# wischmcj/pyQSM

Measured on AMD Instinct MI355X. Metric: Mpoints/s DBSCAN (1M-pt synthetic forest, eps=0.1, min_neighbors=10), higher is better.
Workload: dtype f64; 1 GPU; 1000000-point synthetic tree cloud (configs[1]), DBSCAN eps=0.1 min_neighbors=10, 20 clusters; replicas at N>1; points_per_gpu=1000000, parallelism=replicas x1

## Files before the change

pyqsm_amd/csrc/grid.hip:

```cpp
#include "grid.hpp"

#include <atomic>
#include <cmath>
#include <type_traits>

namespace pyqsm {

__device__ __forceinline__ unsigned long long ord_key(double x) {
  unsigned long long b = static_cast<unsigned long long>(__double_as_longlong(x));
  return (b >> 63) ? ~b : (b | 0x8000000000000000ull);
}
static double ord_val(unsigned long long k) {
  unsigned long long b = (k >> 63) ? (k & 0x7FFFFFFFFFFFFFFFull) : ~k;
  double d;
  memcpy(&d, &b, 8);
  return d;
}

static constexpr int kBoxVals = 7;
__global__ __launch_bounds__(256) void k_bbox(const double* __restrict__ xyz, int64_t n,
                                              unsigned long long* __restrict__ part ,
    unsigned long long* __restrict__ st ) {
  __shared__ unsigned long long red[4][6];
  __shared__ int red_f32[4];
// ... 717 lines not shown
struct BkRec;
template <>
struct BkRec<true> {
  using type = float4;
};
template <>
struct BkRec<false> {
  using type = PointRec;
};

template <int MODE>
__global__ __launch_bounds__(256) void k_bk_hist(const double* __restrict__ xyz, int64_t n, GridParams g,
                                                 int rx, int ry, int rz, AxisMap am, int nbk, int bits,
                                                 int32_t* __restrict__ key_tmp,
                                                 int32_t* __restrict__ tot, const GridPlan* __restrict__ plan) {
  extern __shared__ __attribute__((aligned(16))) int32_t h[];
  if (plan) {
    if (!plan->ok) return;
    g = GridParams{plan->mn[0], plan->mn[1], plan->mn[2], plan->inv_cell, plan->nx, plan->ny, plan->nz};
    rx = plan->rx;
    ry = plan->ry;
    rz = plan->rz;
    nbk = plan->nbk;
    bits = plan->bits;
  }
  for (int b = threadIdx.x; b < nbk; b += 256) h[b] = 0;
  __syncthreads();
  const int64_t base = int64_t(blockIdx.x) * kBkPts;
#pragma unroll
  for (int k = 0; k < kBkPts / 256; ++k) {
    const int64_t i = base + k * 256 + threadIdx.x;
    if (i < n) {
      int c, oct = 0;
      if (MODE == 2) {
        c = cell_index(g, xyz[3 * i], xyz[3 * i + 1], xyz[3 * i + 2]);
      } else {
        const RawCell r = raw_cell(g, rx, ry, rz, xyz[3 * i], xyz[3 * i + 1], xyz[3 * i + 2]);
        const int cx = MODE == 1 ? am.x[r.cx] : r.cx + 1, cy = MODE == 1 ? am.y[r.cy] : r.cy + 1,
                  cz = MODE == 1 ? am.z[r.cz] : r.cz + 1;
        c = (cz * g.ny + cy) * g.nx + cx;
        oct = r.oct;
      }
      key_tmp[i] = (c << 3) | oct;
      atomicAdd(&h[c >> bits], 1);
    }
  }
  __syncthreads();
  for (int b = threadIdx.x; b < nbk; b += 256) {
    const int v = h[b];
    if (v) atomicAdd(&tot[b], v);
  }
}

static constexpr int kBkFusedScan = 4096;
__global__ __launch_bounds__(1024) void k_bk_scan(int nbk, const int32_t* __restrict__ tot,
                                                  int32_t* __restrict__ bstart, const GridPlan* __restrict__ plan) {
  __shared__ int32_t wsum[16];
  if (plan) {
    if (!plan->ok) return;
    nbk = plan->nbk;
  }
  const int per = (nbk + 1023) / 1024;
  const int b0 = threadIdx.x * per;
  int32_t v[16], s = 0;
  for (int k = 0; k < per; ++k) {
    v[k] = b0 + k < nbk ? tot[b0 + k] : 0;
    s += v[k];
  }
  const int lane = threadIdx.x & 63, w = threadIdx.x >> 6;
  int32_t incl = s;
#pragma unroll
  for (int off = 1; off < 64; off <<= 1) {
    const int32_t t = __shfl_up(incl, off, 64);
    if (lane >= off) incl += t;
  }
  if (lane == 63) wsum[w] = incl;
  __syncthreads();
  int32_t run = incl - s;
  for (int q = 0; q < w; ++q) run += wsum[q];
  for (int k = 0; k < per; ++k) {
    if (b0 + k < nbk) bstart[b0 + k] = run;
    run += v[k];
  }
  if (threadIdx.x == 1023) bstart[nbk] = run;
}

template <bool F32>
__global__ __launch_bounds__(256) void k_bk_scatter(const double* __restrict__ xyz, int64_t n, int nbk,
                                                    int bits, const int32_t* __restrict__ key_tmp,
                                                    const int32_t* __restrict__ tot,
                                                    int32_t* __restrict__ cursor ,
                                                    int32_t* __restrict__ bstart ,
                                                    int fused,
                                                    typename BkRec<F32>::type* __restrict__ bucketed,
                                                    int32_t* __restrict__ keyb ,
                                                    const GridPlan* __restrict__ plan) {
  extern __shared__ __attribute__((aligned(16))) int32_t h[];
  const int64_t base = int64_t(blockIdx.x) * kBkPts;
  using Coord = typename std::conditional<F32, float, double>::type;
  int key[kBkPts / 256], lr[kBkPts / 256];
  Coord px[kBkPts / 256], py[kBkPts / 256], pz[kBkPts / 256];
#pragma unroll
  for (int k = 0; k < kBkPts / 256; ++k) {
    const int64_t i = base + k * 256 + threadIdx.x;
    key[k] = -1;
    px[k] = py[k] = pz[k] = Coord(0);
    if (i < n) {
      key[k] = key_tmp[i];
      px[k] = Coord(xyz[3 * i]);
      py[k] = Coord(xyz[3 * i + 1]);
      pz[k] = Coord(xyz[3 * i + 2]);
    }
  }
  if (plan) {
    if (!plan->ok) return;
    nbk = plan->nbk;
    bits = plan->bits;
  }
  int32_t* pre = h + nbk;
  __shared__ int32_t wsum[4];
  for (int b = threadIdx.x; b < nbk; b += 256) h[b] = 0;
  if (fused) {
    constexpr int kPer = kBkFusedScan / 256;
    const int b0 = threadIdx.x * kPer;
    int32_t v[kPer], s = 0;
#pragma unroll
    for (int k = 0; k < kPer; ++k) {
      v[k] = b0 + k < nbk ? tot[b0 + k] : 0;
      s += v[k];
    }
    const int lane = threadIdx.x & 63, w = threadIdx.x >> 6;
    int32_t incl = s;
#pragma unroll
    for (int off = 1; off < 64; off <<= 1) {
      const int32_t t = __shfl_up(incl, off, 64);
      if (lane >= off) incl += t;
    }
    if (lane == 63) wsum[w] = incl;
    __syncthreads();
    int32_t run = incl - s;
    for (int q = 0; q < w; ++q) run += wsum[q];
#pragma unroll
    for (int k = 0; k < kPer; ++k) {
      if (b0 + k < nbk) {
        pre[b0 + k] = run;
        if (blockIdx.x == 0) bstart[b0 + k] = run;
      }
      run += v[k];
    }
    if (blockIdx.x == 0 && threadIdx.x == 255) bstart[nbk] = run;
  }
  __syncthreads();
#pragma unroll
  for (int k = 0; k < kBkPts / 256; ++k) {
    lr[k] = key[k] >= 0 ? atomicAdd(&h[key[k] >> (3 + bits)], 1) : 0;
  }
  __syncthreads();
  for (int bb = 0; bb < nbk; bb += 16 * 256) {
    int32_t v[16], a[16];
#pragma unroll
    for (int k = 0; k < 16; ++k) {
      const int b = bb + k * 256 + threadIdx.x;
      v[k] = b < nbk ? h[b] : 0;
    }
#pragma unroll
    for (int k = 0; k < 16; ++k) {
      a[k] = 0;
      if (v[k]) a[k] = atomicAdd(&cursor[bb + k * 256 + threadIdx.x], v[k]);
    }
#pragma unroll
    for (int k = 0; k < 16; ++k) {
      const int b = bb + k * 256 + threadIdx.x;
      if (v[k]) h[b] = (fused ? pre[b] : bstart[b]) + a[k];
    }
  }
  __syncthreads();
#pragma unroll
  for (int k = 0; k < kBkPts / 256; ++k) {
    if (key[k] < 0) continue;
    const int64_t i = base + k * 256 + threadIdx.x;
    const int pos = h[key[k] >> (3 + bits)] + lr[k];
    keyb[pos] = key[k];
    if constexpr (F32) {
      bucketed[pos] = make_float4(px[k], py[k], pz[k], __int_as_float(int(i)));
    } else {
      PointRec r;
      r.x = px[k];
      r.y = py[k];
      r.z = pz[k];
      r.idx = int(i);
      r.key = key[k];
      bucketed[pos] = r;
    }
  }
}

__device__ __forceinline__ int bytes_below(unsigned long long x, int o) {
  x &= (1ull << (8 * o)) - 1ull;
  x = (x & 0x00FF00FF00FF00FFull) + ((x >> 8) & 0x00FF00FF00FF00FFull);
  x = (x & 0x0000FFFF0000FFFFull) + ((x >> 16) & 0x0000FFFF0000FFFFull);
  return int((x + (x >> 32)) & 0xFFFFull);
}

template <int BITS>
struct BkLds {
  unsigned long long oct[1 << BITS];
  int32_t cnt[1 << BITS];
  uint32_t big[(1 << BITS) / 32];
  int32_t wsum[16];
  int32_t osum[16];
  int32_t any_big;
  int32_t btot[8], bbase[8];
  int32_t bw[(1 << BITS) / 512][8];
};

__device__ __forceinline__ uint32_t bk_word(int lk, int rr, int r8) {
  return (uint32_t(lk) << 16) | (uint32_t(rr < 255 ? rr : 255) << 8) | uint32_t(r8);
}

template <bool F32>
static constexpr int kBkGrp = F32 ? 2 : 1;

template <int BITS, bool F32>
__global__ __launch_bounds__((1 << BITS) / 8, BITS == 12 ? 6 : 4) void k_bk_sort(
    const int32_t* __restrict__ bstart,
    const typename BkRec<F32>::type* __restrict__ bucketed, const int32_t* __restrict__ keyb,
    uint32_t* __restrict__ word_tmp, int32_t* __restrict__ rank_tmp,
    DirWord* __restrict__ words , int32_t* __restrict__ slots ,
    int32_t* __restrict__ order, int32_t* __restrict__ cell_of, int32_t* __restrict__ sub_of,
    double* __restrict__ sx, double* __restrict__ sy, double* __restrict__ sz,
    float4* __restrict__ p4 , int4* __restrict__ rec,
    PointRec* __restrict__ keyed ,
    const GridPlan* __restrict__ plan ,
    unsigned long long* __restrict__ st ) {
  constexpr int CELLS = 1 << BITS, T = CELLS / 8, CAP = T * kBkPer, G = kBkGrp<F32>;
  using Rec = typename BkRec<F32>::type;
  static_assert(kBkPer % G == 0, "whole groups");
  __shared__ BkLds<BITS> L;
  stamped(st, [&] {
  const int bk = blockIdx.x, t = threadIdx.x;
  if (!plan->ok || bk >= plan->nbk) return;
  const int s = bstart[bk], e = bstart[bk + 1];
  const int64_t c0 = int64_t(bk) << BITS;
  constexpr int WORDS = CELLS / 32;
  DirWord* const wds = words + size_t(bk) * WORDS;
  const uint32_t sb = uint32_t(s) + uint32_t(bk);
  if (s == e) {
    if (t < WORDS) wds[t] = DirWord{0u, sb};
    if (t == 0) slots[sb] = s;
    return;
  }
  if (e - s <= 64) {
    int32_t* const cells = L.cnt;
    int32_t* const dcell = L.cnt + 64;
    const int m = e - s;
    if (t < 64) {
      const bool live = t < m;
      const int lk = live ? keyb[s + t] & (8 * CELLS - 1) : 0;
      Rec p = {};
      if (live) p = bucketed[s + t];
      int below_key = 0, below_cell = 0;
      unsigned long long oc = 0ull;
      for (int q = 0; q < m; ++q) {
        const int kq = __builtin_amdgcn_readlane(lk, q);
        below_key += (kq < lk || (kq == lk && q < t)) ? 1 : 0;
        below_cell += (kq >> 3) < (lk >> 3) ? 1 : 0;
        if ((kq >> 3) == (lk >> 3)) oc += 1ull << (8 * (kq & 7));
      }
      if (live) {
        const int cl = lk >> 3, o = lk & 7, b = s + below_cell, f = s + below_key;
        cells[below_key] = cl;
        cell_of[f] = int(c0) + cl;
        sub_of[f] = b * 8 + o;
        if constexpr (F32) {
          order[f] = __float_as_int(p.w);
          p4[f] = make_float4(p.x, p.y, p.z, 0.f);
        } else {
          order[f] = p.idx;
          sx[f] = p.x;
          sy[f] = p.y;
          sz[f] = p.z;
        }
        if (below_key == below_cell) {
          int r2 = b;
#pragma unroll
          for (int o2 = 0; o2 < 8; ++o2) {
            const int cnt = int((oc >> (8 * o2)) & 255ull);
            rec[size_t(b) * 8 + o2] = make_int4(r2, cnt, -1, 0);
            r2 += cnt;
          }
        }
      }
    }
    __syncthreads();
    if (t < 64) {
      const bool live = t < m;
      const int ci = live ? cells[t] : -1;
      const bool head = live && (t == 0 || cells[t - 1] != ci);
      const unsigned long long hm = __ballot(head);
      const int rk = __popcll(hm & ((1ull << t) - 1ull));
      if (head) {
        slots[sb + rk] = s + t;
        dcell[rk] = ci;
      }
      if (t == 0) {
        slots[sb + __popcll(hm)] = e;
        L.wsum[0] = __popcll(hm);
      }
    }
    __syncthreads();
    if (t < WORDS) {
      const int nd = L.wsum[0];
      uint32_t bits = 0u, before = 0u;
      for (int q = 0; q < nd; ++q) {
        const int c = dcell[q];
        before += c < 32 * t ? 1u : 0u;
        bits |= (c >> 5) == t ? 1u << (c & 31) : 0u;
      }
      wds[t] = DirWord{bits, sb + before};
    }
    return;
  }
  uint32_t wd[kBkPer];
#pragma unroll
  for (int k = 0; k < kBkPer; ++k) {
    const int j = s + k * T + t;
    wd[k] = j < e ? uint32_t(keyb[j]) : 0u;
  }
  Rec cur[G] = {};
#pragma unroll
  for (int k = 0; k < G; ++k) {
    const int j = s + k * T + t;
    if (j < e) cur[k] = bucketed[j];
  }
#pragma unroll
  for (int k = 0; k < 8; ++k) {
    L.oct[k * T + t] = 0ull;
    L.cnt[k * T + t] = 0;
  }
  if (t < CELLS / 32) L.big[t] = 0u;
  if (t == 0) L.any_big = 0;
  __syncthreads();
  auto rank_of = [&](uint32_t ky, int j) {
    const int lk = int(ky) & (8 * CELLS - 1), cl = lk >> 3, o = lk & 7;
    const int rr = atomicAdd(&L.cnt[cl], 1);
    const int r8 = int((atomicAdd(&L.oct[cl], 1ull << (8 * o)) >> (8 * o)) & 255ull);
    if (rr >= 255) rank_tmp[j] = rr;
    return bk_word(lk, rr, r8);
  };
#pragma unroll
  for (int k = 0; k < kBkPer; ++k) {
    const int j = s + k * T + t;
    if (j < e) wd[k] = rank_of(wd[k], j);
  }
  for (int base = s + CAP; base < e; base += CAP) {
    uint32_t kk[kBkPer];
#pragma unroll
    for (int k = 0; k < kBkPer; ++k) {
      const int j = base + k * T + t;
      kk[k] = j < e ? uint32_t(keyb[j]) : 0u;
    }
#pragma unroll
    for (int k = 0; k < kBkPer; ++k) {
      const int j = base + k * T + t;
      if (j < e) word_tmp[j] = rank_of(kk[k], j);
    }
  }
  __syncthreads();
  int32_t v[8], tot = 0;
  {
    const int4 a = *reinterpret_cast<const int4*>(&L.cnt[8 * t]);
    const int4 b = *reinterpret_cast<const int4*>(&L.cnt[8 * t + 4]);
    v[0] = a.x; v[1] = a.y; v[2] = a.z; v[3] = a.w;
    v[4] = b.x; v[5] = b.y; v[6] = b.z; v[7] = b.w;
#pragma unroll
    for (int k = 0; k < 8; ++k) tot += v[k];
  }
  uint32_t occ8 = 0u;
#pragma unroll
  for (int k = 0; k < 8; ++k) occ8 |= v[k] ? 1u << k : 0u;
  const int nocc = __popc(occ8);
  const int lane = t & 63, w = t >> 6;
  int32_t incl = tot, oincl = nocc;
#pragma unroll
  for (int off = 1; off < 64; off <<= 1) {
    const int32_t u = __shfl_up(incl, off, 64), uo = __shfl_up(oincl, off, 64);
    if (lane >= off) {
      incl += u;
      oincl += uo;
    }
  }
  if (lane == 63) {
    L.wsum[w] = incl;
    L.osum[w] = oincl;
  }
  __syncthreads();
  int32_t run = incl - tot, orun = oincl - nocc;
  for (int q = 0; q < w; ++q) {
    run += L.wsum[q];
    orun += L.osum[q];
  }
  int32_t pre[8];
#pragma unroll
  for (int k = 0; k < 8; ++k) {
    pre[k] = run;
    run += v[k];
  }
  {
    const uint32_t b1 = __shfl_down(occ8, 1, 64), b2 = __shfl_down(occ8, 2, 64), b3 = __shfl_down(occ8, 3, 64);
    if ((t & 3) == 0) wds[t >> 2] = DirWord{occ8 | (b1 << 8) | (b2 << 16) | (b3 << 24), sb + uint32_t(orun)};
    if (t == T - 1) slots[sb + uint32_t(orun + nocc)] = e;
  }
#pragma unroll
  for (int k = 0; k < 8; ++k) {
    const int cl = 8 * t + k;
    L.cnt[cl] = pre[k];
    if (v[k] == 0) continue;
    const int b = s + pre[k];
    slots[sb + uint32_t(orun) + __popc(occ8 & ((1u << k) - 1u))] = b;
    if (v[k] > kBkBig) {
      atomicOr(&L.big[cl >> 5], 1u << (cl & 31));
      L.any_big = 1;
      continue;
    }
    const unsigned long long c64 = L.oct[cl];
    int r2 = b;
#pragma unroll
    for (int o = 0; o < 8; ++o) {
      const int cnt = int((c64 >> (8 * o)) & 255ull);
      rec[size_t(b) * 8 + o] = make_int4(r2, cnt, -1, 0);
      r2 += cnt;
    }
  }
  __syncthreads();
  auto place = [&](const Rec& p, uint32_t w, int j) {
    const int lk = int(w >> 16), cl = lk >> 3, o = lk & 7, arr = int((w >> 8) & 255u);
    const int b = s + L.cnt[cl];
    if ((L.big[cl >> 5] >> (cl & 31)) & 1u) {
      PointRec q;
      q.x = p.x;
      q.y = p.y;
      q.z = p.z;
      q.key = int(c0 << 3) + lk;
      if constexpr (F32)
        q.idx = __float_as_int(p.w);
      else
        q.idx = p.idx;
      keyed[b + (arr < 255 ? arr : rank_tmp[j])] = q;
      return;
    }
    const int f = b + bytes_below(L.oct[cl], o) + int(w & 255u);
    cell_of[f] = int(c0) + cl;
    sub_of[f] = b * 8 + o;
    if constexpr (F32) {
      order[f] = __float_as_int(p.w);
      p4[f] = make_float4(p.x, p.y, p.z, 0.f);
    } else {
      order[f] = p.idx;
      sx[f] = p.x;
      sy[f] = p.y;
      sz[f] = p.z;
    }
  };
#pragma unroll
  for (int g = 0; g < kBkPer / G; ++g) {
    if (s + g * G * T >= e) break;
    Rec nxt[G] = {};
    if (g + 1 < kBkPer / G) {
#pragma unroll
      for (int k = 0; k < G; ++k) {
        const int j = s + ((g + 1) * G + k) * T + t;
        if (j < e) nxt[k] = bucketed[j];
      }
    }
#pragma unroll
    for (int k = 0; k < G; ++k) {
      const int j = s + (g * G + k) * T + t;
      if (j < e) place(cur[k], wd[g * G + k], j);
    }
#pragma unroll
    for (int k = 0; k < G; ++k) cur[k] = nxt[k];
  }
  for (int base = s + CAP; base < e; base += CAP) {
#pragma unroll
    for (int g = 0; g < kBkPer / G; ++g) {
      if (base + g * G * T >= e) break;
      Rec r[G] = {};
      uint32_t w[G];
#pragma unroll
      for (int k = 0; k < G; ++k) {
        const int j = base + (g * G + k) * T + t;
        w[k] = 0u;
        if (j < e) {
          r[k] = bucketed[j];
          w[k] = word_tmp[j];
        }
      }
#pragma unroll
      for (int k = 0; k < G; ++k) {
        const int j = base + (g * G + k) * T + t;
        if (j < e) place(r[k], w[k], j);
      }
    }
  }
  __syncthreads();
  if (!L.any_big) return;
  for (int wd = 0; wd < CELLS / 32; ++wd) {
    for (uint32_t bm = L.big[wd]; bm; bm &= bm - 1u) {
      const int cl = wd * 32 + __ffs(bm) - 1;
      const int b = s + L.cnt[cl], e2 = s + (cl + 1 < CELLS ? L.cnt[cl + 1] : e - s);
      int loc[8] = {0, 0, 0, 0, 0, 0, 0, 0};
      for (int q = b + t; q < e2; q += T) {
        const int oq = keyed[q].key & 7;
#pragma unroll
        for (int k = 0; k < 8; ++k) loc[k] += oq == k;
      }
      if (t < 8) L.btot[t] = 0;
      __syncthreads();
#pragma unroll
      for (int k = 0; k < 8; ++k) {
        int cnt = loc[k];
        for (int off = 32; off > 0; off >>= 1) cnt += __shfl_down(cnt, off, 64);
        if (lane == 0 && cnt) atomicAdd(&L.btot[k], cnt);
      }
      __syncthreads();
      if (t == 0) {
        int r2 = b;
        for (int k = 0; k < 8; ++k) {
          L.bbase[k] = r2;
          rec[size_t(b) * 8 + k] = make_int4(r2, L.btot[k], -1, 0);
          r2 += L.btot[k];
        }
      }
      __syncthreads();
      for (int q0 = b; q0 < e2; q0 += T) {
        const int q = q0 + t;
        const bool live = q < e2;
        PointRec pr;
        pr.key = 0;
        if (live) pr = keyed[q];
        const int o = pr.key & 7;
        int before = 0;
#pragma unroll
        for (int k = 0; k < 8; ++k) {
          const unsigned long long m = __ballot(live && o == k);
          if (lane == 0) L.bw[w][k] = __popcll(m);
          if (o == k) before = __popcll(m & ((1ull << lane) - 1ull));
        }
        __syncthreads();
        if (live) {
          int f = L.bbase[o] + before;
          for (int ww = 0; ww < w; ++ww) f += L.bw[ww][o];
          order[f] = pr.idx;
          cell_of[f] = pr.key >> 3;
          sub_of[f] = b * 8 + o;
          if (p4) {
            p4[f] = make_float4(float(pr.x), float(pr.y), float(pr.z), 0.f);
          } else {
            sx[f] = pr.x;
            sy[f] = pr.y;
            sz[f] = pr.z;
          }
        }
        __syncthreads();
        if (t < 8) {
          int add = 0;
          for (int ww = 0; ww < T / 64; ++ww) add += L.bw[ww][t];
          L.bbase[t] += add;
        }
        __syncthreads();
      }
    }
  }
  });
}

template <int BITS, bool F32>
__global__ __launch_bounds__((1 << BITS) / 8, BITS == 12 ? 6 : 4) void k_bk_sort_plain(
    int64_t ncell1, const int32_t* __restrict__ bstart, const typename BkRec<F32>::type* __restrict__ bucketed,
    const int32_t* __restrict__ keyb, uint32_t* __restrict__ word_tmp, int32_t* __restrict__ rank_tmp,
    int32_t* __restrict__ start, int32_t* __restrict__ order,
    int32_t* __restrict__ cell_of, double* __restrict__ sx, double* __restrict__ sy, double* __restrict__ sz,
    float4* __restrict__ p4 , int32_t* __restrict__ occ) {
  constexpr int CELLS = 1 << BITS, T = CELLS / 8, CAP = T * kBkPer, G = kBkGrp<F32>;
  using Rec = typename BkRec<F32>::type;
  __shared__ int32_t cnt[CELLS];
  __shared__ int32_t wsum[16], wocc[16];
  const int bk = blockIdx.x, t = threadIdx.x;
  const int s = bstart[bk], e = bstart[bk + 1];
  const int64_t c0 = int64_t(bk) << BITS;
  if (s == e) {
#pragma unroll
    for (int k = 0; k < 2; ++k) {
      const int64_t cidx = c0 + int64_t(k * T + t) * 4;
      if (cidx + 3 < ncell1) {
        *reinterpret_cast<int4*>(start + cidx) = make_int4(s, s, s, s);
      } else {
        for (int u = 0; u < 4; ++u)
          if (cidx + u < ncell1) start[cidx + u] = s;
      }
    }
    if (t == 0) occ[bk] = 0;
    return;
  }
  constexpr int RB = 32 - BITS;
  constexpr int RMAX = (1 << RB) - 1;
  uint32_t wd[kBkPer];
#pragma unroll
  for (int k = 0; k < kBkPer; ++k) {
    const int j = s + k * T + t;
    wd[k] = j < e ? uint32_t(keyb[j]) : 0u;
  }
  Rec cur[G] = {};
#pragma unroll
  for (int k = 0; k < G; ++k) {
    const int j = s + k * T + t;
    if (j < e) cur[k] = bucketed[j];
  }
#pragma unroll
  for (int k = 0; k < 8; ++k) cnt[k * T + t] = 0;
  __syncthreads();
  auto rank_of = [&](uint32_t ky, int j) {
    const int cl = int(ky >> 3) & (CELLS - 1);
    const int rr = atomicAdd(&cnt[cl], 1);
    if (rr >= RMAX) rank_tmp[j] = rr;
    return (uint32_t(cl) << RB) | uint32_t(rr < RMAX ? rr : RMAX);
// ... 84 lines not shown
  };
#pragma unroll
  for (int g = 0; g < kBkPer / G; ++g) {
    if (s + g * G * T >= e) break;
    Rec nxt[G] = {};
    if (g + 1 < kBkPer / G) {
#pragma unroll
      for (int k = 0; k < G; ++k) {
        const int j = s + ((g + 1) * G + k) * T + t;
        if (j < e) nxt[k] = bucketed[j];
      }
    }
#pragma unroll
    for (int k = 0; k < G; ++k) {
      const int j = s + (g * G + k) * T + t;
      if (j < e) place(cur[k], wd[g * G + k], j);
    }
#pragma unroll
    for (int k = 0; k < G; ++k) cur[k] = nxt[k];
  }
  for (int base = s + CAP; base < e; base += CAP) {
#pragma unroll
    for (int g = 0; g < kBkPer / G; ++g) {
      if (base + g * G * T >= e) break;
      Rec r[G] = {};
      uint32_t w[G];
#pragma unroll
      for (int k = 0; k < G; ++k) {
        const int j = base + (g * G + k) * T + t;
        w[k] = 0u;
        if (j < e) {
          r[k] = bucketed[j];
          w[k] = word_tmp[j];
        }
      }
#pragma unroll
      for (int k = 0; k < G; ++k) {
        const int j = base + (g * G + k) * T + t;
        if (j < e) place(r[k], w[k], j);
      }
    }
  }
}

static bool bucketed_fits(const DevGrid& g) {
  const int bits = g.ncell + 1 <= (int64_t(kBkMax) << 12) ? 12 : 13;
  const int64_t nbk = (g.ncell + (int64_t(1) << bits)) >> bits;
  const char* env = getenv("PYQSM_GRID_BIN");
  return nbk <= kBkMax && !(env && !strcmp(env, "atomic"));
}

static void enqueue_bk_a(Ctx* c, int mode, bool f32, const double* xyz, int64_t n, const GridParams& gp,
                         const int raw[3], AxisMap am, int64_t nbk, int bits, int32_t* key_tmp, int32_t* tot,
                         int32_t* cursor, int32_t* bstart, void* bucketed, int32_t* keyb, const GridPlan* d_plan) {
  const dim3 ga(ceil_div(n, kBkPts)), blk(256);
  const size_t lds = size_t(nbk) * 4;
  const int fused = nbk <= kBkFusedScan;
#define PQ_BK_HIST(MODE)                                                                                         \
  hipLaunchKernelGGL(k_bk_hist<MODE>, ga, blk, lds, c->stream, xyz, n, gp, raw[0], raw[1], raw[2], am, int(nbk), \
                     bits, key_tmp, tot, d_plan)
  if (mode == 0)
    PQ_BK_HIST(0);
  else if (mode == 1)
    PQ_BK_HIST(1);
  else
    PQ_BK_HIST(2);
#undef PQ_BK_HIST
  if (!fused) hipLaunchKernelGGL(k_bk_scan, dim3(1), dim3(1024), 0, c->stream, int(nbk), tot, bstart, d_plan);
  if (f32)
    hipLaunchKernelGGL(k_bk_scatter<true>, ga, blk, fused ? 2 * lds : lds, c->stream, xyz, n, int(nbk), bits,
                       key_tmp, tot, cursor, bstart, fused, static_cast<float4*>(bucketed), keyb, d_plan);
  else
    hipLaunchKernelGGL(k_bk_scatter<false>, ga, blk, fused ? 2 * lds : lds, c->stream, xyz, n, int(nbk), bits,
                       key_tmp, tot, cursor, bstart, fused, static_cast<PointRec*>(bucketed), keyb, d_plan);
}

template <int BITS, bool F32>
static void launch_bk_sort_plain(Ctx* c, int64_t nbk, const int32_t* bstart, const void* bucketed, const int32_t* keyb,
                                 uint32_t* word_tmp, int32_t* rank_tmp, DevGrid* g) {
  hipLaunchKernelGGL((k_bk_sort_plain<BITS, F32>), dim3(unsigned(nbk)), dim3((1 << BITS) / 8), 0, c->stream,
                     g->ncell + 1, bstart, static_cast<const typename BkRec<F32>::type*>(bucketed), keyb, word_tmp,
                     rank_tmp, g->start, g->order, g->cell_of, g->sx, g->sy, g->sz, g->p4, g->occ_part);
}

static int build_grid_bucketed(Ctx* c, const double* xyz, int64_t n, DevGrid* g) {
  const int bits = g->ncell + 1 <= (int64_t(kBkMax) << 12) ? 12 : 13;
  const int64_t nbk = (g->ncell + (int64_t(1) << bits)) >> bits;
  const bool f32 = g->p4 != nullptr;
  int32_t *tot, *bstart, *cursor, *key_tmp, *keyb, *rank_tmp;
  uint32_t* word_tmp;
  void* bucketed;
  PQ_TRY(c->arena.get(size_t(nbk) * 2, &tot));
  cursor = tot + nbk;
  PQ_TRY(c->arena.get(size_t(nbk) + 1, &bstart));
  PQ_TRY(c->arena.get(size_t(n), &key_tmp));
  PQ_TRY(c->arena.get(size_t(n), &keyb));
  PQ_TRY(c->arena.get(size_t(n), &word_tmp));
  PQ_TRY(c->arena.get(size_t(n), &rank_tmp));
  if (f32) {
    float4* b4;
    PQ_TRY(c->arena.get(size_t(n), &b4));
    bucketed = b4;
  } else {
    PointRec* b8;
    PQ_TRY(c->arena.get(size_t(n), &b8));
    bucketed = b8;
  }
  g->occ_blocks = int(nbk);
  PQ_TRY(c->arena.get(size_t(nbk), &g->occ_part));
  PQ_HIP(hipMemsetAsync(tot, 0, size_t(nbk) * 8, c->stream));
  const int raw[3] = {0, 0, 0};
  enqueue_bk_a(c, 2, f32, xyz, n, grid_params(*g), raw, AxisMap{nullptr, nullptr, nullptr}, nbk, bits, key_tmp, tot,
               cursor, bstart, bucketed, keyb, nullptr);
  if (bits == 12) {
    if (f32)
      launch_bk_sort_plain<12, true>(c, nbk, bstart, bucketed, keyb, word_tmp, rank_tmp, g);
    else
      launch_bk_sort_plain<12, false>(c, nbk, bstart, bucketed, keyb, word_tmp, rank_tmp, g);
  } else {
    if (f32)
      launch_bk_sort_plain<13, true>(c, nbk, bstart, bucketed, keyb, word_tmp, rank_tmp, g);
    else
      launch_bk_sort_plain<13, false>(c, nbk, bstart, bucketed, keyb, word_tmp, rank_tmp, g);
  }
  PQ_HIP(hipGetLastError());
  return 0;
}


__device__ __forceinline__ double ord_val_dev(unsigned long long k) {
  const unsigned long long b = (k >> 63) ? (k & 0x7FFFFFFFFFFFFFFFull) : ~k;
  return __longlong_as_double(static_cast<long long>(b));
}

__device__ void write_plan(const unsigned long long* box, const PlanIn& in, GridPlan* __restrict__ plan) {
  GridPlan p;
  bool ok = in.hint.valid != 0;
  for (int a = 0; a < 3; ++a) {
    p.mn[a] = ord_val_dev(box[a]);
    p.mx[a] = ord_val_dev(box[3 + a]);
    ok = ok && isfinite(p.mn[a]) && isfinite(p.mx[a]);
  }
  p.all_f32 = box[6] != 0 ? 1 : 0;
  ok = ok && p.all_f32;
  double tot = 1.0;
  int raw[3];
  for (int a = 0; a < 3; ++a) {
    const double d = floor((p.mx[a] - p.mn[a]) / in.cell) + 1.0;
    if (!(d < 2.0e9)) ok = false;
    raw[a] = ok ? int(d) : 0;
    tot *= d + 2.0;
  }
  ok = ok && tot <= double(in.max_cells);
  p.inv_cell = 1.0 / in.cell;
  p.rx = raw[0];
  p.ry = raw[1];
  p.rz = raw[2];
  p.nx = raw[0] + 2;
  p.ny = raw[1] + 2;
  p.nz = raw[2] + 2;
  const int64_t ncell = ok ? int64_t(p.nx) * p.ny * p.nz : 0;
  const int64_t nbk = (ncell + 4096) >> 12;
  ok = ok && ncell + 1 <= (int64_t(kBkMax) << 12) && ncell <= in.hint.ncell && nbk <= in.hint.nbk &&
       (nbk <= kBkFusedScan) == (in.hint.fused != 0);
  p.ncell = ok ? int(ncell) : 0;
  p.nbk = ok ? int(nbk) : 0;
  p.bits = 12;
  p.ok = ok ? 1 : 0;
  p.seq = in.seq;
  *plan = p;
  if (in.host) {
    p.seq = 0;
    *in.host = p;
    __threadfence_system();
    *reinterpret_cast<volatile unsigned*>(&in.host->seq) = in.seq;
  }
}

int plan_grid_device(Ctx* c, const double* xyz, int64_t n, double cell, int64_t max_cells, const PlanHint& hint,
                     GridPlan* d_plan, GridPlan* h_plan, unsigned seq, int32_t* zero_buf, int zero_n) {
  if (n <= 0) return fail(PYQSM_EINVAL, "bounding box of an empty cloud");
  const int blocks = int(std::min<int64_t>(ceil_div(n, 256), int64_t(c->cu_count) * 4));
  unsigned long long *d_box = nullptr, *d_part = nullptr;
  PQ_TRY(c->arena.get(kBoxVals, &d_box));
  PQ_TRY(c->arena.get(size_t(blocks) * kBoxVals, &d_part));
  hipLaunchKernelGGL(k_bbox, dim3(blocks), dim3(256), 0, c->stream, xyz, n, d_part, stamp_slots(c, blocks));
  hipLaunchKernelGGL(k_bbox_fold, dim3(1), dim3(256), 0, c->stream, d_part, blocks, d_box, zero_buf, zero_n,
                     PlanIn{cell, max_cells, hint, h_plan, seq}, d_plan);
  PQ_HIP(hipGetLastError());
  return 0;
}

int octant_zeroed_ints() { return 2 * kBkMax + 5 + kZeroedExtra; }

template <int BITS, bool F32>
static void launch_bk_sort(Ctx* c, int64_t nbk, const int32_t* bstart, const void* bucketed,
                           const int32_t* keyb, uint32_t* word_tmp, int32_t* rank_tmp, PointRec* keyed,
                           const GridPlan* d_plan, DevGrid* g, SubCells* sub) {
  unsigned long long* const st_sort = stamp_slots(c, nbk);
  hipLaunchKernelGGL((k_bk_sort<BITS, F32>), dim3(unsigned(nbk)), dim3((1 << BITS) / 8), 0, c->stream, bstart,
                     static_cast<const typename BkRec<F32>::type*>(bucketed), keyb, word_tmp, rank_tmp, g->dir_words,
                     g->dir_slots, g->order,
                     g->cell_of, sub->sub_of, g->sx, g->sy, g->sz, g->p4, sub->rec, keyed, d_plan, st_sort);
}

static int enqueue_bucketed(Ctx* c, const double* xyz, int64_t n, const GridParams& gp, const int raw[3],
                            AxisMap am, bool mapped, int64_t nbk, int bits, bool f32,
                            int32_t* zeroed, const GridPlan* d_plan, DevGrid* g, SubCells* sub) {
  int32_t *cell_tmp, *keyb, *rank_tmp, *bstart;
  uint32_t* word_tmp;
  int32_t *tot = zeroed, *cursor = zeroed + kBkMax;
  PointRec* keyed;
  void* bucketed;
  g->p4 = nullptr;
  g->sx = g->sy = g->sz = nullptr;
  sub->sub_cnt = sub->sub_beg = nullptr;
  g->start = nullptr;
  PQ_TRY(c->arena.get(size_t(nbk) << (bits - 5), &g->dir_words));
  PQ_TRY(c->arena.get(size_t(n) + size_t(nbk) + 1, &g->dir_slots));
  PQ_TRY(c->arena.get(size_t(n), &g->order));
  PQ_TRY(c->arena.get(size_t(n), &g->cell_of));
  if (f32) {
    float4* b4;
    PQ_TRY(c->arena.get(size_t(n), &g->p4));
    PQ_TRY(c->arena.get(size_t(n), &b4));
    bucketed = b4;
  } else {
    PointRec* b8;
    PQ_TRY(c->arena.get(size_t(n), &g->sx));
    PQ_TRY(c->arena.get(size_t(n), &g->sy));
    PQ_TRY(c->arena.get(size_t(n), &g->sz));
    PQ_TRY(c->arena.get(size_t(n), &b8));
    bucketed = b8;
  }
  PQ_TRY(c->arena.get(size_t(n), &cell_tmp));
  PQ_TRY(c->arena.get(size_t(n), &keyb));
  PQ_TRY(c->arena.get(size_t(n), &word_tmp));
  PQ_TRY(c->arena.get(size_t(n), &rank_tmp));
  PQ_TRY(c->arena.get(size_t(n), &keyed));
  PQ_TRY(c->arena.get(size_t(n), &sub->sub_of));
  PQ_TRY(c->arena.get(size_t(n) * 8, &sub->rec));
  PQ_TRY(c->arena.get(size_t(nbk) + 1, &bstart));
  enqueue_bk_a(c, mapped ? 1 : 0, f32, xyz, n, gp, raw, am, nbk, bits, cell_tmp, tot, cursor, bstart, bucketed, keyb,
               d_plan);
  if (bits == 12) {
    if (f32)
      launch_bk_sort<12, true>(c, nbk, bstart, bucketed, keyb, word_tmp, rank_tmp, keyed, d_plan, g, sub);
    else
      launch_bk_sort<12, false>(c, nbk, bstart, bucketed, keyb, word_tmp, rank_tmp, keyed, d_plan, g, sub);
  } else {
    if (f32)
      launch_bk_sort<13, true>(c, nbk, bstart, bucketed, keyb, word_tmp, rank_tmp, keyed, d_plan, g, sub);
    else
      launch_bk_sort<13, false>(c, nbk, bstart, bucketed, keyb, word_tmp, rank_tmp, keyed, d_plan, g, sub);
  }
  PQ_HIP(hipGetLastError());
  return 0;
}

__global__ __launch_bounds__(256) void k_dir_from_dense(int64_t ncell, const int32_t* __restrict__ start,
                                                        DirWord* __restrict__ words, int32_t* __restrict__ slots) {
  const int64_t c = int64_t(blockIdx.x) * 256 + threadIdx.x;
  const int lane = threadIdx.x & 63, half = lane >> 5;
  const int a = start[c < ncell ? c : ncell];
  const int b = start[c + 1 < ncell ? c + 1 : ncell];
  const uint32_t bits = uint32_t(__ballot(b != a) >> (32 * half));
  const int64_t w = c >> 5;
  const uint32_t base = uint32_t(__shfl(a, half * 32, 64)) + uint32_t(w);
  if (w > (ncell >> 5)) return;
  if (b != a) slots[base + __popc(bits & ((1u << (lane & 31)) - 1u))] = a;
  if ((lane & 31) == 31) slots[base + __popc(bits)] = b;
  if ((lane & 31) == 0) words[w] = DirWord{bits, base};
}

static int dir_from_dense(Ctx* c, int64_t n, DevGrid* g) {
  const int64_t nwords = (g->ncell >> 5) + 1;
  PQ_TRY(c->arena.get(size_t(nwords), &g->dir_words));
  PQ_TRY(c->arena.get(size_t(n) + size_t(nwords) + 1, &g->dir_slots));
  hipLaunchKernelGGL(k_dir_from_dense, dim3(unsigned(ceil_div(nwords * 32, 256))), dim3(256), 0, c->stream, g->ncell,
                     g->start, g->dir_words, g->dir_slots);
  PQ_HIP(hipGetLastError());
  return 0;
}

__global__ __launch_bounds__(256) void k_read_directory(int64_t ncell, const CellDir dir,
                                                        int32_t* __restrict__ out) {
  const int64_t c = int64_t(blockIdx.x) * 256 + threadIdx.x;
  if (c <= ncell) out[c] = dir.begin(int(c));
}

void read_directory(Ctx* c, const DevGrid& g, int64_t ncell, int32_t* begin_out) {
  hipLaunchKernelGGL(k_read_directory, dim3(unsigned(ceil_div(ncell + 1, 256))), dim3(256), 0, c->stream, ncell,
                     cell_dir(g), begin_out);
}

int bin_octants_planned(Ctx* c, const double* xyz, int64_t n, double cell, const PlanHint& hint,
                        const GridPlan* d_plan, int32_t* zeroed, DevGrid* g, SubCells* sub) {
  g->minx = g->miny = g->minz = 0.0;
  g->cell = cell;
  g->inv_cell = 1.0 / cell;
  g->nx = g->ny = g->nz = 0;
  g->ncell = hint.ncell;
  sub->zeroed4 = zeroed + 2 * kBkMax + 1;
  const int raw[3] = {0, 0, 0};
  return enqueue_bucketed(c, xyz, n, GridParams{}, raw, AxisMap{nullptr, nullptr, nullptr}, false, hint.nbk, 12,
                          true, zeroed, d_plan, g, sub);
}
// ... 409 lines not shown
```

Before: 3428 Mpoints/s.

## Split bucket sort into persistent heavy blocks and per-wave light bucket workers

The scan kernels now classify buckets as heavy (more than 64 points) or light and write compact lists of each. k_bk_sort launches a fixed-size grid: the first ga blocks loop persistently over heavy buckets with the next bucket bounds prefetched, and the remaining blocks give each wave its own light or empty bucket, instead of one full block per bucket. This removes the cost of launching one block per bucket, most of which sit idle on tiny buckets. Smaller tweaks add 32-bit index addressing, an unrolled predicated wave-sum loop and a constexpr F32 branch; in exchange the code is more complex and grid sizing relies on a CU-count heuristic with an env override.

```diff
diff --git a/pyqsm_amd/csrc/grid.hip b/pyqsm_amd/csrc/grid.hip
--- a/pyqsm_amd/csrc/grid.hip
+++ b/pyqsm_amd/csrc/grid.hip
@@ -793,37 +793,68 @@
   }
 }
 
+static constexpr int kBkLight = 64;
+__device__ __forceinline__ void bk_list_put(int32_t* __restrict__ lists, int cap, int b, int32_t total,
+                                            int32_t& before) {
+  if (total > kBkLight)
+    lists[2 + before++] = b;
+  else
+    lists[2 + cap + b - before] = b;
+}
+
 static constexpr int kBkFusedScan = 4096;
 __global__ __launch_bounds__(1024) void k_bk_scan(int nbk, const int32_t* __restrict__ tot,
-                                                  int32_t* __restrict__ bstart, const GridPlan* __restrict__ plan) {
-  __shared__ int32_t wsum[16];
+                                                  int32_t* __restrict__ bstart,
+                                                  int32_t* __restrict__ lists ,
+                                                  const GridPlan* __restrict__ plan) {
+  __shared__ int32_t wsum[16], hsum[16];
+  const int cap = nbk;
   if (plan) {
     if (!plan->ok) return;
     nbk = plan->nbk;
   }
   const int per = (nbk + 1023) / 1024;
   const int b0 = threadIdx.x * per;
-  int32_t v[16], s = 0;
+  int32_t v[16], s = 0, hv = 0;
   for (int k = 0; k < per; ++k) {
     v[k] = b0 + k < nbk ? tot[b0 + k] : 0;
     s += v[k];
+    hv += v[k] > kBkLight ? 1 : 0;
   }
   const int lane = threadIdx.x & 63, w = threadIdx.x >> 6;
-  int32_t incl = s;
+  int32_t incl = s, hincl = hv;
 #pragma unroll
   for (int off = 1; off < 64; off <<= 1) {
-    const int32_t t = __shfl_up(incl, off, 64);
-    if (lane >= off) incl += t;
-  }
-  if (lane == 63) wsum[w] = incl;
-  __syncthreads();
-  int32_t run = incl - s;
-  for (int q = 0; q < w; ++q) run += wsum[q];
+    const int32_t t = __shfl_up(incl, off, 64), th = __shfl_up(hincl, off, 64);
+    if (lane >= off) {
+      incl += t;
+      hincl += th;
+    }
+  }
+  if (lane == 63) {
+    wsum[w] = incl;
+    hsum[w] = hincl;
+  }
+  __syncthreads();
+  int32_t run = incl - s, hrun = hincl - hv;
+  for (int q = 0; q < w; ++q) {
+    run += wsum[q];
+    hrun += hsum[q];
+  }
   for (int k = 0; k < per; ++k) {
-    if (b0 + k < nbk) bstart[b0 + k] = run;
+    if (b0 + k < nbk) {
+      bstart[b0 + k] = run;
+      if (lists) bk_list_put(lists, cap, b0 + k, v[k], hrun);
+    }
     run += v[k];
   }
-  if (threadIdx.x == 1023) bstart[nbk] = run;
+  if (threadIdx.x == 1023) {
+    bstart[nbk] = run;
+    if (lists) {
+      lists[0] = hrun;
+      lists[1] = nbk - hrun;
+    }
+  }
 }
 
 template <bool F32>
@@ -833,6 +864,7 @@
                                                     int32_t* __restrict__ cursor ,
                                                     int32_t* __restrict__ bstart ,
                                                     int fused,
+                                                    int32_t* __restrict__ lists ,
                                                     typename BkRec<F32>::type* __restrict__ bucketed,
                                                     int32_t* __restrict__ keyb ,
                                                     const GridPlan* __restrict__ plan) {
@@ -853,13 +885,14 @@
       pz[k] = Coord(xyz[3 * i + 2]);
     }
   }
+  const int cap = nbk;
   if (plan) {
     if (!plan->ok) return;
     nbk = plan->nbk;
     bits = plan->bits;
   }
   int32_t* pre = h + nbk;
-  __shared__ int32_t wsum[4];
+  __shared__ int32_t wsum[4], hsum[4];
   for (int b = threadIdx.x; b < nbk; b += 256) h[b] = 0;
   if (fused) {
     constexpr int kPer = kBkFusedScan / 256;
@@ -878,18 +911,41 @@
       if (lane >= off) incl += t;
     }
     if (lane == 63) wsum[w] = incl;
+    const bool listing = blockIdx.x == 0 && lists != nullptr;
+    int32_t hv = 0, hincl = 0;
+    if (listing) {
+#pragma unroll
+      for (int k = 0; k < kPer; ++k) hv += v[k] > kBkLight ? 1 : 0;
+      hincl = hv;
+#pragma unroll
+      for (int off = 1; off < 64; off <<= 1) {
+        const int32_t t = __shfl_up(hincl, off, 64);
+        if (lane >= off) hincl += t;
+      }
+      if (lane == 63) hsum[w] = hincl;
+    }
     __syncthreads();
-    int32_t run = incl - s;
+    int32_t run = incl - s, hrun = hincl - hv;
     for (int q = 0; q < w; ++q) run += wsum[q];
+    if (listing) {
+      for (int q = 0; q < w; ++q) hrun += hsum[q];
+    }
 #pragma unroll
     for (int k = 0; k < kPer; ++k) {
       if (b0 + k < nbk) {
         pre[b0 + k] = run;
         if (blockIdx.x == 0) bstart[b0 + k] = run;
+        if (listing) bk_list_put(lists, cap, b0 + k, v[k], hrun);
       }
       run += v[k];
     }
-    if (blockIdx.x == 0 && threadIdx.x == 255) bstart[nbk] = run;
+    if (blockIdx.x == 0 && threadIdx.x == 255) {
+      bstart[nbk] = run;
+      if (listing) {
+        lists[0] = hrun;
+        lists[1] = nbk - hrun;
+      }
+    }
   }
   __syncthreads();
 #pragma unroll
@@ -955,6 +1011,12 @@
   int32_t bw[(1 << BITS) / 512][8];
 };
 
+template <typename P>
+__device__ __forceinline__ P& at32(P* base, int i) {
+  return *reinterpret_cast<P*>(reinterpret_cast<char*>(const_cast<std::remove_const_t<P>*>(base)) +
+                               size_t(uint32_t(i) * uint32_t(sizeof(P))));
+}
+
 __device__ __forceinline__ uint32_t bk_word(int lk, int rr, int r8) {
   return (uint32_t(lk) << 16) | (uint32_t(rr < 255 ? rr : 255) << 8) | uint32_t(r8);
 }
@@ -963,48 +1025,50 @@
 static constexpr int kBkGrp = F32 ? 2 : 1;
 
 template <int BITS, bool F32>
-__global__ __launch_bounds__((1 << BITS) / 8, BITS == 12 ? 6 : 4) void k_bk_sort(
-    const int32_t* __restrict__ bstart,
+__device__ __forceinline__ void bk_sort_light(
+    int32_t* lds, const int32_t* __restrict__ bstart, const int32_t* __restrict__ lists, int cap, int ga,
     const typename BkRec<F32>::type* __restrict__ bucketed, const int32_t* __restrict__ keyb,
-    uint32_t* __restrict__ word_tmp, int32_t* __restrict__ rank_tmp,
-    DirWord* __restrict__ words , int32_t* __restrict__ slots ,
-    int32_t* __restrict__ order, int32_t* __restrict__ cell_of, int32_t* __restrict__ sub_of,
-    double* __restrict__ sx, double* __restrict__ sy, double* __restrict__ sz,
-    float4* __restrict__ p4 , int4* __restrict__ rec,
-    PointRec* __restrict__ keyed ,
-    const GridPlan* __restrict__ plan ,
-    unsigned long long* __restrict__ st ) {
-  constexpr int CELLS = 1 << BITS, T = CELLS / 8, CAP = T * kBkPer, G = kBkGrp<F32>;
+    DirWord* __restrict__ words, int32_t* __restrict__ slots, int32_t* __restrict__ order,
+    int32_t* __restrict__ cell_of, int32_t* __restrict__ sub_of, double* __restrict__ sx, double* __restrict__ sy,
+    double* __restrict__ sz, float4* __restrict__ p4, int4* __restrict__ rec) {
+  constexpr int CELLS = 1 << BITS, T = CELLS / 8, WORDS = CELLS / 32;
   using Rec = typename BkRec<F32>::type;
-  static_assert(kBkPer % G == 0, "whole groups");
-  __shared__ BkLds<BITS> L;
-  stamped(st, [&] {
-  const int bk = blockIdx.x, t = threadIdx.x;
-  if (!plan->ok || bk >= plan->nbk) return;
-  const int s = bstart[bk], e = bstart[bk + 1];
-  const int64_t c0 = int64_t(bk) << BITS;
-  constexpr int WORDS = CELLS / 32;
-  DirWord* const wds = words + size_t(bk) * WORDS;
-  const uint32_t sb = uint32_t(s) + uint32_t(bk);
-  if (s == e) {
-    if (t < WORDS) wds[t] = DirWord{0u, sb};
-    if (t == 0) slots[sb] = s;
-    return;
-  }
-  if (e - s <= 64) {
-    int32_t* const cells = L.cnt;
-    int32_t* const dcell = L.cnt + 64;
+  const int t = threadIdx.x;
+  constexpr int WAVES = T / 64;
+  static_assert(WAVES * 128 <= CELLS, "a slice per wave inside L.cnt");
+  const int lane = t & 63, wv = t >> 6;
+  const int nwave = (int(gridDim.x) - ga) * WAVES;
+  int32_t* const cells = lds + wv * 128;
+  int32_t* const dcell = cells + 64;
+  const auto wave_sync = [] {
+    __builtin_amdgcn_fence(__ATOMIC_RELEASE, "wavefront");
+    __builtin_amdgcn_wave_barrier();
+    __builtin_amdgcn_fence(__ATOMIC_ACQUIRE, "wavefront");
+  };
+  const int nl = lists[1];
+  for (int i = __builtin_amdgcn_readfirstlane((int(blockIdx.x) - ga) * WAVES + wv); i < nl; i += nwave) {
+    const int bk = __builtin_amdgcn_readfirstlane(lists[2 + cap + i]);
+    const int s = __builtin_amdgcn_readfirstlane(bstart[bk]), e = __builtin_amdgcn_readfirstlane(bstart[bk + 1]);
+    const int64_t c0 = int64_t(bk) << BITS;
+    DirWord* const wds = words + size_t(bk) * WORDS;
+    const uint32_t sb = uint32_t(s) + uint32_t(bk);
     const int m = e - s;
-    if (t < 64) {
-      const bool live = t < m;
-      const int lk = live ? keyb[s + t] & (8 * CELLS - 1) : 0;
+    if (m == 0) {
+#pragma unroll
+      for (int q = lane; q < WORDS; q += 64) wds[q] = DirWord{0u, sb};
+      if (lane == 0) slots[sb] = s;
+      continue;
+    }
+    const bool live = lane < m;
+    {
+      const int lk = live ? keyb[s + lane] & (8 * CELLS - 1) : 0;
       Rec p = {};
-      if (live) p = bucketed[s + t];
+      if (live) p = bucketed[s + lane];
       int below_key = 0, below_cell = 0;
       unsigned long long oc = 0ull;
       for (int q = 0; q < m; ++q) {
         const int kq = __builtin_amdgcn_readlane(lk, q);
-        below_key += (kq < lk || (kq == lk && q < t)) ? 1 : 0;
+        below_key += (kq < lk || (kq == lk && q < lane)) ? 1 : 0;
         below_cell += (kq >> 3) < (lk >> 3) ? 1 : 0;
         if ((kq >> 3) == (lk >> 3)) oc += 1ull << (8 * (kq & 7));
       }
@@ -1033,60 +1097,90 @@
         }
       }
     }
-    __syncthreads();
-    if (t < 64) {
-      const bool live = t < m;
-      const int ci = live ? cells[t] : -1;
-      const bool head = live && (t == 0 || cells[t - 1] != ci);
-      const unsigned long long hm = __ballot(head);
-      const int rk = __popcll(hm & ((1ull << t) - 1ull));
-      if (head) {
-        slots[sb + rk] = s + t;
-        dcell[rk] = ci;
-      }
-      if (t == 0) {
-        slots[sb + __popcll(hm)] = e;
-        L.wsum[0] = __popcll(hm);
-      }
-    }
-    __syncthreads();
-    if (t < WORDS) {
-      const int nd = L.wsum[0];
+    wave_sync();
+    const int ci = live ? cells[lane] : -1;
+    const bool head = live && (lane == 0 || cells[lane - 1] != ci);
+    const unsigned long long hm = __ballot(head);
+    const int nd = __popcll(hm);
+    const int rk = __popcll(hm & ((1ull << lane) - 1ull));
+    if (head) {
+      slots[sb + rk] = s + lane;
+      dcell[rk] = ci;
+    }
+    if (lane == 0) slots[sb + nd] = e;
+    wave_sync();
+#pragma unroll
+    for (int wq = lane; wq < WORDS; wq += 64) {
       uint32_t bits = 0u, before = 0u;
       for (int q = 0; q < nd; ++q) {
         const int c = dcell[q];
-        before += c < 32 * t ? 1u : 0u;
-        bits |= (c >> 5) == t ? 1u << (c & 31) : 0u;
+        before += c < 32 * wq ? 1u : 0u;
+        bits |= (c >> 5) == wq ? 1u << (c & 31) : 0u;
       }
-      wds[t] = DirWord{bits, sb + before};
-    }
+      wds[wq] = DirWord{bits, sb + before};
+    }
+    wave_sync();
+  }
+}
+
+template <int BITS, bool F32>
+__global__ __launch_bounds__((1 << BITS) / 8, BITS == 12 ? 6 : 4) void k_bk_sort(
+    const int32_t* __restrict__ bstart, const int32_t* __restrict__ lists , int cap ,
+    int ga ,
+    const typename BkRec<F32>::type* __restrict__ bucketed, const int32_t* __restrict__ keyb,
+    uint32_t* __restrict__ word_tmp, int32_t* __restrict__ rank_tmp,
+    DirWord* __restrict__ words , int32_t* __restrict__ slots ,
+    int32_t* __restrict__ order, int32_t* __restrict__ cell_of, int32_t* __restrict__ sub_of,
+    double* __restrict__ sx, double* __restrict__ sy, double* __restrict__ sz,
+    float4* __restrict__ p4 , int4* __restrict__ rec,
+    PointRec* __restrict__ keyed ,
+    const GridPlan* __restrict__ plan, unsigned long long* __restrict__ st ) {
+  constexpr int CELLS = 1 << BITS, T = CELLS / 8, CAP = T * kBkPer, G = kBkGrp<F32>;
+  using Rec = typename BkRec<F32>::type;
+  static_assert(kBkPer % G == 0, "whole groups");
+  __shared__ BkLds<BITS> L;
+  stamped(st, [&] {
+  if (!plan->ok) return;
+  constexpr int WORDS = CELLS / 32;
+  if (int(blockIdx.x) >= ga) {
+    bk_sort_light<BITS, F32>(L.cnt, bstart, lists, cap, ga, bucketed, keyb, words, slots, order, cell_of, sub_of, sx,
+                             sy, sz, p4, rec);
     return;
   }
+  const int nh = lists[0];
+  const auto heavy_bucket = [&](const int bk, const int s, const int e) {
+  int t = threadIdx.x;
+  unsigned long long zero64 = 0ull;
+  asm volatile("" : "+v"(t), "+v"(zero64));
+  const int64_t c0 = int64_t(bk) << BITS;
+  DirWord* const wds = words + size_t(bk) * WORDS;
+  const uint32_t sb = uint32_t(s) + uint32_t(bk);
   uint32_t wd[kBkPer];
 #pragma unroll
   for (int k = 0; k < kBkPer; ++k) {
     const int j = s + k * T + t;
-    wd[k] = j < e ? uint32_t(keyb[j]) : 0u;
+    wd[k] = j < e ? uint32_t(at32(keyb, j)) : 0u;
   }
   Rec cur[G] = {};
 #pragma unroll
   for (int k = 0; k < G; ++k) {
     const int j = s + k * T + t;
-    if (j < e) cur[k] = bucketed[j];
+    if (j < e) cur[k] = at32(bucketed, j);
   }
 #pragma unroll
   for (int k = 0; k < 8; ++k) {
-    L.oct[k * T + t] = 0ull;
+    L.oct[k * T + t] = zero64;
     L.cnt[k * T + t] = 0;
   }
   if (t < CELLS / 32) L.big[t] = 0u;
   if (t == 0) L.any_big = 0;
   __syncthreads();
+  asm volatile("" : "+v"(t));
   auto rank_of = [&](uint32_t ky, int j) {
     const int lk = int(ky) & (8 * CELLS - 1), cl = lk >> 3, o = lk & 7;
     const int rr = atomicAdd(&L.cnt[cl], 1);
     const int r8 = int((atomicAdd(&L.oct[cl], 1ull << (8 * o)) >> (8 * o)) & 255ull);
-    if (rr >= 255) rank_tmp[j] = rr;
+    if (rr >= 255) at32(rank_tmp, j) = rr;
     return bk_word(lk, rr, r8);
   };
 #pragma unroll
@@ -1099,12 +1193,12 @@
 #pragma unroll
     for (int k = 0; k < kBkPer; ++k) {
       const int j = base + k * T + t;
-      kk[k] = j < e ? uint32_t(keyb[j]) : 0u;
+      kk[k] = j < e ? uint32_t(at32(keyb, j)) : 0u;
     }
 #pragma unroll
     for (int k = 0; k < kBkPer; ++k) {
       const int j = base + k * T + t;
-      if (j < e) word_tmp[j] = rank_of(kk[k], j);
+      if (j < e) at32(word_tmp, j) = rank_of(kk[k], j);
     }
   }
   __syncthreads();
@@ -1137,9 +1231,11 @@
   }
   __syncthreads();
   int32_t run = incl - tot, orun = oincl - nocc;
-  for (int q = 0; q < w; ++q) {
-    run += L.wsum[q];
-    orun += L.osum[q];
+#pragma unroll
+  for (int q = 0; q < T / 64 - 1; ++q) {
+    const int32_t ws = L.wsum[q], os = L.osum[q];
+    run += q < w ? ws : 0;
+    orun += q < w ? os : 0;
   }
   int32_t pre[8];
 #pragma unroll
@@ -1174,6 +1270,7 @@
     }
   }
   __syncthreads();
+  asm volatile("" : "+v"(t));
   auto place = [&](const Rec& p, uint32_t w, int j) {
     const int lk = int(w >> 16), cl = lk >> 3, o = lk & 7, arr = int((w >> 8) & 255u);
     const int b = s + L.cnt[cl];
@@ -1187,20 +1284,20 @@
         q.idx = __float_as_int(p.w);
       else
         q.idx = p.idx;
-      keyed[b + (arr < 255 ? arr : rank_tmp[j])] = q;
+      keyed[b + (arr < 255 ? arr : at32(rank_tmp, j))] = q;
       return;
     }
     const int f = b + bytes_below(L.oct[cl], o) + int(w & 255u);
-    cell_of[f] = int(c0) + cl;
-    sub_of[f] = b * 8 + o;
+    at32(cell_of, f) = int(c0) + cl;
+    at32(sub_of, f) = b * 8 + o;
     if constexpr (F32) {
-      order[f] = __float_as_int(p.w);
-      p4[f] = make_float4(p.x, p.y, p.z, 0.f);
+      at32(order, f) = __float_as_int(p.w);
+      at32(p4, f) = make_float4(p.x, p.y, p.z, 0.f);
     } else {
-      order[f] = p.idx;
-      sx[f] = p.x;
-      sy[f] = p.y;
-      sz[f] = p.z;
+      at32(order, f) = p.idx;
+      at32(sx, f) = p.x;
+      at32(sy, f) = p.y;
+      at32(sz, f) = p.z;
     }
   };
 #pragma unroll
@@ -1211,7 +1308,7 @@
 #pragma unroll
       for (int k = 0; k < G; ++k) {
         const int j = s + ((g + 1) * G + k) * T + t;
-        if (j < e) nxt[k] = bucketed[j];
+        if (j < e) nxt[k] = at32(bucketed, j);
       }
     }
 #pragma unroll
@@ -1233,8 +1330,8 @@
         const int j = base + (g * G + k) * T + t;
         w[k] = 0u;
         if (j < e) {
-          r[k] = bucketed[j];
-          w[k] = word_tmp[j];
+          r[k] = at32(bucketed, j);
+          w[k] = at32(word_tmp, j);
         }
       }
 #pragma unroll
@@ -1295,7 +1392,7 @@
           order[f] = pr.idx;
           cell_of[f] = pr.key >> 3;
           sub_of[f] = b * 8 + o;
-          if (p4) {
+          if constexpr (F32) {
             p4[f] = make_float4(float(pr.x), float(pr.y), float(pr.z), 0.f);
           } else {
             sx[f] = pr.x;
@@ -1313,6 +1410,23 @@
       }
     }
   }
+  };
+  int i = blockIdx.x;
+  if (i >= nh) return;
+  int bk = lists[2 + i], bk1 = i + ga < nh ? lists[2 + i + ga] : bk;
+  int s = bstart[bk], e = bstart[bk + 1];
+  for (;;) {
+    const int bk2 = i + 2 * ga < nh ? lists[2 + i + 2 * ga] : bk1;
+    const int s1 = bstart[bk1], e1 = bstart[bk1 + 1];
+    heavy_bucket(bk, s, e);
+    i += ga;
+    if (i >= nh) break;
+    bk = bk1;
+    bk1 = bk2;
+    s = s1;
+    e = e1;
+    __syncthreads();
+  }
   });
 }
 
@@ -1503,7 +1617,8 @@
 
 static void enqueue_bk_a(Ctx* c, int mode, bool f32, const double* xyz, int64_t n, const GridParams& gp,
                          const int raw[3], AxisMap am, int64_t nbk, int bits, int32_t* key_tmp, int32_t* tot,
-                         int32_t* cursor, int32_t* bstart, void* bucketed, int32_t* keyb, const GridPlan* d_plan) {
+                         int32_t* cursor, int32_t* bstart, int32_t* lists ,
+                         void* bucketed, int32_t* keyb, const GridPlan* d_plan) {
   const dim3 ga(ceil_div(n, kBkPts)), blk(256);
   const size_t lds = size_t(nbk) * 4;
   const int fused = nbk <= kBkFusedScan;
@@ -1517,13 +1632,14 @@
   else
     PQ_BK_HIST(2);
 #undef PQ_BK_HIST
-  if (!fused) hipLaunchKernelGGL(k_bk_scan, dim3(1), dim3(1024), 0, c->stream, int(nbk), tot, bstart, d_plan);
+  if (!fused)
+    hipLaunchKernelGGL(k_bk_scan, dim3(1), dim3(1024), 0, c->stream, int(nbk), tot, bstart, lists, d_plan);
   if (f32)
     hipLaunchKernelGGL(k_bk_scatter<true>, ga, blk, fused ? 2 * lds : lds, c->stream, xyz, n, int(nbk), bits,
-                       key_tmp, tot, cursor, bstart, fused, static_cast<float4*>(bucketed), keyb, d_plan);
+                       key_tmp, tot, cursor, bstart, fused, lists, static_cast<float4*>(bucketed), keyb, d_plan);
   else
     hipLaunchKernelGGL(k_bk_scatter<false>, ga, blk, fused ? 2 * lds : lds, c->stream, xyz, n, int(nbk), bits,
-                       key_tmp, tot, cursor, bstart, fused, static_cast<PointRec*>(bucketed), keyb, d_plan);
+                       key_tmp, tot, cursor, bstart, fused, lists, static_cast<PointRec*>(bucketed), keyb, d_plan);
 }
 
 template <int BITS, bool F32>
@@ -1562,7 +1678,7 @@
   PQ_HIP(hipMemsetAsync(tot, 0, size_t(nbk) * 8, c->stream));
   const int raw[3] = {0, 0, 0};
   enqueue_bk_a(c, 2, f32, xyz, n, grid_params(*g), raw, AxisMap{nullptr, nullptr, nullptr}, nbk, bits, key_tmp, tot,
-               cursor, bstart, bucketed, keyb, nullptr);
+               cursor, bstart, nullptr, bucketed, keyb, nullptr);
   if (bits == 12) {
     if (f32)
       launch_bk_sort_plain<12, true>(c, nbk, bstart, bucketed, keyb, word_tmp, rank_tmp, g);
@@ -1645,11 +1761,21 @@
 int octant_zeroed_ints() { return 2 * kBkMax + 5 + kZeroedExtra; }
 
 template <int BITS, bool F32>
-static void launch_bk_sort(Ctx* c, int64_t nbk, const int32_t* bstart, const void* bucketed,
+static void launch_bk_sort(Ctx* c, int64_t nbk, const int32_t* bstart, const int32_t* lists, const void* bucketed,
                            const int32_t* keyb, uint32_t* word_tmp, int32_t* rank_tmp, PointRec* keyed,
                            const GridPlan* d_plan, DevGrid* g, SubCells* sub) {
-  unsigned long long* const st_sort = stamp_slots(c, nbk);
-  hipLaunchKernelGGL((k_bk_sort<BITS, F32>), dim3(unsigned(nbk)), dim3((1 << BITS) / 8), 0, c->stream, bstart,
+  constexpr int kWaves = (1 << BITS) / 512;
+  int64_t ga = std::min<int64_t>(nbk, int64_t(c->cu_count) * (BITS == 12 ? 6 : 2));
+  int64_t gb = std::min<int64_t>(ceil_div(nbk, kWaves), ga);
+  if (const char* e_grid = getenv("PYQSM_BK_SORT_GRID")) {
+    const char* comma = strchr(e_grid, ',');
+    const int64_t a = atoi(e_grid), b = comma ? atoi(comma + 1) : 0;
+    if (a > 0) ga = std::min<int64_t>(a, kBkMax);
+    if (b > 0) gb = std::min<int64_t>(b, kBkMax);
+  }
+  unsigned long long* const st_sort = stamp_slots(c, ga + gb);
+  hipLaunchKernelGGL((k_bk_sort<BITS, F32>), dim3(unsigned(ga + gb)), dim3((1 << BITS) / 8), 0, c->stream, bstart,
+                     lists, int(nbk), int(ga),
                      static_cast<const typename BkRec<F32>::type*>(bucketed), keyb, word_tmp, rank_tmp, g->dir_words,
                      g->dir_slots, g->order,
                      g->cell_of, sub->sub_of, g->sx, g->sy, g->sz, g->p4, sub->rec, keyed, d_plan, st_sort);
@@ -1658,7 +1784,7 @@
 static int enqueue_bucketed(Ctx* c, const double* xyz, int64_t n, const GridParams& gp, const int raw[3],
                             AxisMap am, bool mapped, int64_t nbk, int bits, bool f32,
                             int32_t* zeroed, const GridPlan* d_plan, DevGrid* g, SubCells* sub) {
-  int32_t *cell_tmp, *keyb, *rank_tmp, *bstart;
+  int32_t *cell_tmp, *keyb, *rank_tmp, *bstart, *lists;
   uint32_t* word_tmp;
   int32_t *tot = zeroed, *cursor = zeroed + kBkMax;
   PointRec* keyed;
@@ -1692,18 +1818,19 @@
   PQ_TRY(c->arena.get(size_t(n), &sub->sub_of));
   PQ_TRY(c->arena.get(size_t(n) * 8, &sub->rec));
   PQ_TRY(c->arena.get(size_t(nbk) + 1, &bstart));
-  enqueue_bk_a(c, mapped ? 1 : 0, f32, xyz, n, gp, raw, am, nbk, bits, cell_tmp, tot, cursor, bstart, bucketed, keyb,
-               d_plan);
+  PQ_TRY(c->arena.get(2 * size_t(nbk) + 2, &lists));
+  enqueue_bk_a(c, mapped ? 1 : 0, f32, xyz, n, gp, raw, am, nbk, bits, cell_tmp, tot, cursor, bstart, lists, bucketed,
+               keyb, d_plan);
   if (bits == 12) {
     if (f32)
-      launch_bk_sort<12, true>(c, nbk, bstart, bucketed, keyb, word_tmp, rank_tmp, keyed, d_plan, g, sub);
+      launch_bk_sort<12, true>(c, nbk, bstart, lists, bucketed, keyb, word_tmp, rank_tmp, keyed, d_plan, g, sub);
     else
-      launch_bk_sort<12, false>(c, nbk, bstart, bucketed, keyb, word_tmp, rank_tmp, keyed, d_plan, g, sub);
+      launch_bk_sort<12, false>(c, nbk, bstart, lists, bucketed, keyb, word_tmp, rank_tmp, keyed, d_plan, g, sub);
   } else {
     if (f32)
-      launch_bk_sort<13, true>(c, nbk, bstart, bucketed, keyb, word_tmp, rank_tmp, keyed, d_plan, g, sub);
+      launch_bk_sort<13, true>(c, nbk, bstart, lists, bucketed, keyb, word_tmp, rank_tmp, keyed, d_plan, g, sub);
     else
-      launch_bk_sort<13, false>(c, nbk, bstart, bucketed, keyb, word_tmp, rank_tmp, keyed, d_plan, g, sub);
+      launch_bk_sort<13, false>(c, nbk, bstart, lists, bucketed, keyb, word_tmp, rank_tmp, keyed, d_plan, g, sub);
   }
   PQ_HIP(hipGetLastError());
   return 0;
```

Measured after the change: 3436 Mpoints/s, median of 5. Within noise of the previous version (+0.2%).
